# Linyou/Ced-NeRF

Measured on NVIDIA B200. Metric: train_step_rays_per_s, higher is better.
Workload: dtype f16 (MLP, tables) / f32 (marching, compositing, grads)

## Files before the change

cednerf_b200/_lib.py:

```python
from __future__ import annotations

import ctypes
import os
from typing import Optional

import torch

_HERE = os.path.dirname(os.path.abspath(__file__))
LIB_PATH = os.environ.get("CEDNERF_B200_LIB") or os.path.join(_HERE, "libcednerf_b200.so")

MAX_LEVELS = 32
MLP_MAX_LAYERS = 5


class GridLevels(ctypes.Structure):
    _fields_ = [("n_levels", ctypes.c_int), ("scale", ctypes.c_float * MAX_LEVELS),
                ("res", ctypes.c_uint32 * MAX_LEVELS), ("size", ctypes.c_uint32 * MAX_LEVELS),
                ("offset", ctypes.c_uint32 * MAX_LEVELS), ("hashed", ctypes.c_uint32 * MAX_LEVELS)]


class MlpDesc(ctypes.Structure):
    _fields_ = [("n_layers", ctypes.c_int), ("dim_in", ctypes.c_int * MLP_MAX_LAYERS),
                ("dim_out", ctypes.c_int * MLP_MAX_LAYERS), ("param_off", ctypes.c_int * MLP_MAX_LAYERS),
                ("image_off", ctypes.c_int * MLP_MAX_LAYERS), ("image_bytes", ctypes.c_int)]
# ... 39 lines not shown
class DpSmall(ctypes.Structure):
    _fields_ = [("world", ctypes.c_int), ("n_tensors", ctypes.c_int), ("grad", ctypes.c_void_p * DP_MAX_RANKS),
                ("p", ctypes.c_void_p * 8), ("m", ctypes.c_void_p * 8), ("v", ctypes.c_void_p * 8),
                ("off", ctypes.c_int64 * 8), ("n", ctypes.c_int64 * 8), ("lr", ctypes.c_float * 8),
                ("weight_decay", ctypes.c_float * 8), ("grad_div", ctypes.c_float), ("chunk_begin", ctypes.c_int64 * 9)]


class RenderRound(ctypes.Structure):
    _P, _I, _L, _F = ctypes.c_void_p, ctypes.c_int, ctypes.c_int64, ctypes.c_float
    _fields_ = [("rays_o", _P), ("rays_d", _P), ("n_rays", _L), ("occ_bits", _P), ("aabbs", _P), ("n_levels", _I),
                ("resolution", _I), ("near_term", _P), ("far_const", _F), ("step_size", _F), ("cone_angle", _F),
                ("early_stop_eps", _F), ("t_sorted", _P), ("t_indices", _P), ("hits", _P), ("state", _P), ("total", _P),
                ("n_samples", _P), ("run_t", _P), ("run_n", _P), ("n_runs", _P), ("occ_coarse", _P), ("capacity", _L),
                ("offsets", _P), ("totals", _P), ("scan_workspace", _P), ("t_starts", _P), ("t_ends", _P),
                ("ray_indices", _P), ("overflow", _P), ("timestamps", _P), ("image_deform", _P), ("image_density", _P),
                ("image_colour", _P), ("table_f16", _P), ("desc", ctypes.POINTER(FieldDesc)), ("sigma", _P), ("rgbs", _P),
                ("colors", _P), ("opacity", _P), ("depth", _P), ("alive_flags", _P), ("positions", _P),
                ("position_totals", _P), ("run_cap", _I), ("k_hint", _I), ("max_samples", _I), ("min_samples", _I)]


_SIGNATURES = {
    "cednerf_ray_aabb_intersect": "pplpifffpppp",
    "cednerf_sort_boundaries": "pplippp",
    "cednerf_occ_pack_bits": "plpp",
    "cednerf_occ_threshold_pack": "plpppp",
    "cednerf_occ_mark_invisible": "pipiipiiiifpp",
    "cednerf_march": "ipplppiippffffippppppppppppppppppppppippp",
    "cednerf_occ_coarsen": "piipp",
    "cednerf_ray_coherence_keys": "plpp",
    "cednerf_ray_coherence_order": "plppp",
    "cednerf_march_fill_runs": "lppppiffppppp",
    "cednerf_exclusive_scan": "plppppp",
    "cednerf_exclusive_scan_capped": "pllpppp",
    "cednerf_march_fill_runs_capped": "lpppppiffppppp",
    "cednerf_compact_samples_capped": "pppppllpppp",
    "cednerf_hashgrid_fwd": "pilpGpip",
    "cednerf_hashgrid_bwd": "pilpGpiippp",
    "cednerf_hashgrid_bwd_table_lm": "pilGppp",
    "cednerf_hashgrid4d_fwd": "pilpGpiip",
    "cednerf_hashgrid4d_bwd": "pilGpiipip",
    "cednerf_cast_f32_to_f16": "pplp",
    "cednerf_frequency_fwd": "pilipiifp",
    "cednerf_frequency_bwd": "pilipiipp",
    "cednerf_sh2_fwd": "plpip",
    "cednerf_time_embed": "pplpp",
    "cednerf_mlp_pack_weights": "pMpp",
    "cednerf_mlp_fwd": "ppMlppp",
    "cednerf_mlp_bwd": "ppppMlpippp",
    "cednerf_field_fwd": "ppppppppilppppFpppp",
    "cednerf_occ_update_level": "plpppiffpppFpppp",
    "cednerf_field_train_fwd": "ppppppilpppppFppppppppp",
    "cednerf_field_train_bwd": "ppppppilpppppFpppppppppppppippp",
    "cednerf_sample_order": "ppppplpffffffppp",
    "cednerf_ray_offsets": "pllpp",
    "cednerf_composite_fwd": "pppppppillpppppppifp",
    "cednerf_composite_bwd": "pppppppillppppppppppfp",
    "cednerf_visibility_mask": "ppppllffppp",
    "cednerf_compact_samples": "pppppllpppp",
    "cednerf_accumulate_fwd": "ppipllpip",
    "cednerf_accumulate_bwd": "ppiplppppp",
    "cednerf_render_round_begin": "pliippp",
    "cednerf_march_round": "ipplppiipfffppppppppppppppipp",
    "cednerf_march_fill_runs_round": "lpppppiffppppppp",
    "cednerf_render_round_composite": "pppppppplifppppp",
    "cednerf_render_round_compact":"ppplppliippp",
    "cednerf_render_round": "Rlppp",
    "cednerf_generate_rays": "ppppiffffiilpppp",
    "cednerf_distortion_fwd": "pppplpppp",
    "cednerf_distortion_bwd": "pppplpppp",
    "cednerf_importance_keys": "ppplpp",
    "cednerf_topk_select": "pllpppp",
    "cednerf_importance_batch": "pliiippiffffipppppppp",
    "cednerf_nonfinite_check": "App",
    "cednerf_training_loss_fwd": "ppplppplpiffpppp",
    "cednerf_training_loss_bwd": "pppplpppliffpppppp",
    "cednerf_adam_step": "Apippfffip",
    "cednerf_peer_alloc": "lp",
    "cednerf_peer_free": "p",
    "cednerf_ipc_export": "pp",
    "cednerf_ipc_open": "pp",
    "cednerf_ipc_close": "p",
    "cednerf_dp_barrier": "Puip",
    "cednerf_dp_found_inf": "Pppp",
    "cednerf_dp_adam": "Dpppfffip",
    "cednerf_dp_adam_small": "Spppfffip",
}
_CT = {"p": ctypes.c_void_p, "i": ctypes.c_int, "l": ctypes.c_int64, "f": ctypes.c_float,
       "G": ctypes.POINTER(GridLevels), "M": ctypes.POINTER(MlpDesc), "F": ctypes.POINTER(FieldDesc),
       "A": ctypes.POINTER(AdamTensors), "P": ctypes.POINTER(DpPeers), "D": ctypes.POINTER(DpAdam), "S": ctypes.POINTER(DpSmall),
       "u": ctypes.c_uint32, "R": ctypes.POINTER(RenderRound)}

_lib = None


def load() -> ctypes.CDLL:
    global _lib
    if _lib is not None:
        return _lib
    if not os.path.exists(LIB_PATH):
        raise ImportError(
            f"{LIB_PATH} is missing: build it with `make -C cednerf_b200/csrc` (or `python -c 'import "
            "__graft_entry__ as g; g.build()'`).  cednerf_b200 has no CPU / PyTorch fallback.")
    lib = ctypes.CDLL(LIB_PATH)
    lib.cednerf_last_error.restype = ctypes.c_char_p
    lib.cednerf_scan_workspace_bytes.restype = ctypes.c_int64
    lib.cednerf_launch_count.restype = ctypes.c_int64
# ... 78 lines not shown
```

cednerf_b200/csrc/field_train.cu:

```cuda
#include <stdlib.h>

#include "field_common.cuh"

namespace {

struct SavedLayout {
  int64_t h1, o1, in2, h2, o2, h3, h4, o4, xn, total, tiles;
};

__host__ __device__ inline SavedLayout saved_layout(const CednerfFieldDesc& d, int64_t n) {
  SavedLayout s;
  int64_t off = 0;
  const int64_t tiles = (n + MLP_TILE - 1) / MLP_TILE;
  s.tiles = tiles;
  s.h1 = off, off += (int64_t)(d.f1.n_layers - 1) * tiles * MLP_TILE_BYTES;
  s.o1 = off, off += n * 32;
  s.in2 = off, off += n * d.f2.dim_in[0] * 2;
  s.h2 = off, off += (int64_t)(d.f2.n_layers - 1) * tiles * MLP_TILE_BYTES;
  s.o2 = off, off += n * 32;
  s.h3 = off, off += (int64_t)(d.f3.n_layers - 1) * tiles * MLP_TILE_BYTES;
  s.h4 = off, off += d.f4.n_layers > 0 ? (int64_t)(d.f4.n_layers - 1) * tiles * MLP_TILE_BYTES : 0;
  s.o4 = off, off += d.f4.n_layers > 0 ? n * 64 : 0;
  s.xn = off, off += (n * 12 + 15) / 16 * 16;
  s.total = off;
  return s;
}

struct BwdWorkLayout {
  int64_t d_o2, d_in2, d_in4, g_xn, dy_lm, total;
};

__host__ __device__ inline BwdWorkLayout bwd_layout(const CednerfFieldDesc& d, int64_t n) {
  BwdWorkLayout w;
  int64_t off = 0;
  w.d_o2 = off, off += n * 32;
  w.d_in2 = off, off += n * d.f2.dim_in[0] * 2;
  w.d_in4 = off, off += n * 64;
  w.g_xn = off, off += (n * 12 + 15) / 16 * 16;
  w.dy_lm = off, off += (int64_t)d.levels.n_levels * n * 4;
  w.total = off;
  return w;
}

struct TrainArgs {
  const int64_t* ridx;
  const float* t0;
  const float* t1;
  const float* rays_o;
  const float* rays_d;
  const float* t;
  int t_stride;
  int64_t n;
  const int64_t* n_dev;
  const uint8_t* img[4];
  const __half* table;
  float* sigma;
  float* rgb;
  float* latent;
  uint8_t* selector;
  float* move;
  uint8_t* saved;
  const float* d_sigma;
  const float* d_rgb;
  const float* d_latent;
  uint8_t* work;
  float* d_params[4];
  uint32_t tmem_cols;
  int flush_tiles;
  const int32_t* order;
  CednerfFieldDesc d;
};

__device__ __forceinline__ int64_t ext_index(const TrainArgs& a, int64_t s) { return a.order ? (int64_t)a.order[s] : s; }

__device__ __forceinline__ int64_t live_count(const TrainArgs& a) {
  if (!a.n_dev) return a.n;
  const int64_t v = *a.n_dev;
  return v < a.n ? v : a.n;
}

__device__ __forceinline__ float huber(float x) {
  const float ax = fabsf(x);
  return ax < 1.f ? 0.5f * x * x : ax - 0.5f;
}

__device__ __forceinline__ void load_off(const TrainArgs& a, const SavedLayout& sl, int64_t s, float* off6) {
  const uint4 w = *reinterpret_cast<const uint4*>(a.saved + sl.o1 + s * 32);
  const uint32_t ww[4] = {w.x, w.y, w.z, w.w};
#pragma unroll
// ... 27 lines not shown
__global__ void __launch_bounds__(TRAIN_FWD_GROUPS * 128, 1) field_train_fwd_kernel(TrainArgs a) {
  extern __shared__ __align__(1024) uint8_t smem_raw[];
  uint8_t* smem = reinterpret_cast<uint8_t*>((reinterpret_cast<uintptr_t>(smem_raw) + 1023) & ~(uintptr_t)1023);
  const CednerfFieldDesc& d = a.d;
  const bool has4 = d.f4.n_layers > 0;
  const int n_groups = blockDim.x / MLP_TILE;
  const int tid = threadIdx.x, warp = tid >> 5, group = tid / MLP_TILE, gtid = tid % MLP_TILE;
  uint8_t* w1 = smem;
  uint8_t* w2 = w1 + d.f1.image_bytes;
  uint8_t* w3 = w2 + d.f2.image_bytes;
  uint8_t* w4 = w3 + d.f3.image_bytes;
  uint8_t* abuf = reinterpret_cast<uint8_t*>(
                      (reinterpret_cast<uintptr_t>(w4 + (has4 ? d.f4.image_bytes : 0)) + 1023) & ~(uintptr_t)1023) +
                  (size_t)group * MLP_TILE_BYTES;
  __shared__ uint64_t bars[8];
  __shared__ uint32_t tmem_base_s;
  uint64_t* bar = &bars[group];
  {
    const uint8_t* src[4] = {a.img[0], a.img[1], a.img[2], a.img[3]};
    uint8_t* dst[4] = {w1, w2, w3, w4};
    const int bytes[4] = {d.f1.image_bytes, d.f2.image_bytes, d.f3.image_bytes, has4 ? d.f4.image_bytes : 0};
    for (int k = 0; k < 4; ++k)
      for (int q = tid; q < bytes[k] / 16; q += blockDim.x)
        reinterpret_cast<uint4*>(dst[k])[q] = __ldg(reinterpret_cast<const uint4*>(src[k]) + q);
  }
  const uint32_t tmem_cols = n_groups <= 1 ? 64 : (n_groups == 2 ? 128 : (n_groups <= 4 ? 256 : 512));
  if (warp == 0) tmem_alloc(&tmem_base_s, tmem_cols);
  if (gtid == 0) mbar_init(bar, 1);
  if (tid == 0) fence_barrier_init();
  fence_proxy_async();
  tc_fence_before();
  __syncthreads();
  tc_fence_after();
  const uint32_t tmem_base = tmem_base_s + 64u * (uint32_t)group;
  const uint32_t tmem_warp = tmem_base + ((uint32_t)((warp & 3) * 32) << 16);
  uint32_t phase = 0;
  const int64_t n = a.n, nl = live_count(a);
  const int64_t n_tiles = (nl + MLP_TILE - 1) / MLP_TILE;
  const int L = d.levels.n_levels;
  const uint32_t one2 = 0x3C003C00u;
  const SavedLayout sl = saved_layout(d, n);
  const int k2 = d.f2.dim_in[0];

  for (int64_t tile = blockIdx.x + (int64_t)gridDim.x * group; tile < n_tiles; tile += (int64_t)gridDim.x * n_groups) {
    const int64_t s = tile * MLP_TILE + gtid;
    const bool ok = s < nl;
    const int rows_valid = (int)((nl - tile * MLP_TILE) < MLP_TILE ? (nl - tile * MLP_TILE) : MLP_TILE);
    float x[3] = {0.f, 0.f, 0.f}, tv = 0.f;
    int64_t ray = 0;
#ifdef FIELD_PHASE_CLOCKS
    long long phase_t = clock64();
    if (gtid == 0) atomicAdd(&g_train_phase_clocks[11], 1ull);
#endif
    const int64_t e = ok ? ext_index(a, s) : 0;
    if (ok) packed_sample(a.ridx, a.t0, a.t1, a.rays_o, a.rays_d, a.t, a.t_stride, e, x, tv, ray);
    frequency_row<true>(abuf, gtid, x[0], x[1], x[2], tv);
    fence_proxy_async();
    tc_fence_before();
    group_sync(group);
    TPHASE_MARK(0);
    run_chain(d.f1, w1, abuf, tmem_base, tmem_warp, bar, phase, gtid, group, a.saved + sl.h1,
              sl.tiles, tile * MLP_TILE, rows_valid);
    TPHASE_MARK(1);
    float xn[3], mv[3], mvnorm;
    bool selector;
    {
      uint32_t r[16];
      tmem_ld16(tmem_warp, r);
      tmem_ld_wait();
      uint32_t p[8];
#pragma unroll
      for (int j = 0; j < 8; ++j) p[j] = pack_h2(__uint_as_float(r[2 * j]), __uint_as_float(r[2 * j + 1]));
      if (ok) {
        uint4* dst = reinterpret_cast<uint4*>(a.saved + sl.o1 + s * 32);
        dst[0] = make_uint4(p[0], p[1], p[2], p[3]);
        dst[1] = make_uint4(p[4], p[5], p[6], p[7]);
      }
      float off6[6];
#pragma unroll
      for (int k = 0; k < 6; ++k) off6[k] = rnd16(r[k]);
      apply_move(d, x, off6, mv, xn, selector);
      mvnorm = sqrtf(mv[0] * mv[0] + mv[1] * mv[1] + mv[2] * mv[2]);
    }
    if (ok) {
      float* xs = reinterpret_cast<float*>(a.saved + sl.xn) + 3 * s;
      xs[0] = xn[0], xs[1] = xn[1], xs[2] = xn[2];
      a.move[3 * e] = mv[0], a.move[3 * e + 1] = mv[1], a.move[3 * e + 2] = mv[2];
      a.selector[e] = (uint8_t)selector;
    }
    TPHASE_MARK(2);
    float temb[9];
    {
      auto put_word = [&](int w, uint32_t v) {
        *reinterpret_cast<uint32_t*>(abuf + swz(gtid, w >> 2) + ((w & 3) << 2)) = v;
      };
      if ((L % TRAIN_FWD_LG) == 0 && (L & 3) == 0) {
#pragma unroll 1
        for (int l0 = 0; l0 < L; l0 += TRAIN_FWD_LG) {
          uint32_t fw[TRAIN_FWD_LG];
          hash_levels<TRAIN_FWD_LG>(xn, a.table, d.levels, 0, fw, l0);
          if constexpr (TRAIN_FWD_LG >= 4) {
#pragma unroll
            for (int q = 0; q < TRAIN_FWD_LG / 4; ++q)
              *reinterpret_cast<uint4*>(abuf + swz(gtid, (l0 >> 2) + q)) = make_uint4(fw[4 * q], fw[4 * q + 1], fw[4 * q + 2], fw[4 * q + 3]);
          } else {
            *reinterpret_cast<uint2*>(abuf + swz(gtid, l0 >> 2) + ((l0 & 2) << 2)) = make_uint2(fw[0], fw[1]);
          }
        }
// ... 117 lines not shown
__device__ __forceinline__ void predictor_dout(const TrainArgs& a, const SavedLayout& sl, int64_t s, int cb, uint32_t* dw) {
  const int k2 = a.d.f2.dim_in[0];
  const uint4* ps = reinterpret_cast<const uint4*>(a.saved + sl.o4 + s * 64) + 2 * cb;
  const uint4* fs = reinterpret_cast<const uint4*>(a.saved + sl.in2 + s * k2 * 2) + 2 * cb;
  const int64_t e = ext_index(a, s);
  const bool sel = a.selector[e] != 0;
#pragma unroll
  for (int c = 0; c < 2; ++c) {
    const uint4 p = ps[c], f = fs[c];
    const uint32_t pw[4] = {p.x, p.y, p.z, p.w}, fw[4] = {f.x, f.y, f.z, f.w};
    const float4 l0 = *reinterpret_cast<const float4*>(a.d_latent + e * 32 + (2 * cb + c) * 8);
    const float4 l1 = *reinterpret_cast<const float4*>(a.d_latent + e * 32 + (2 * cb + c) * 8 + 4);
    const float lg[8] = {l0.x, l0.y, l0.z, l0.w, l1.x, l1.y, l1.z, l1.w};
#pragma unroll
    for (int j = 0; j < 4; ++j) {
      const float2 pv = __half22float2(*reinterpret_cast<const __half2*>(&pw[j]));
      const float2 fv = __half22float2(*reinterpret_cast<const __half2*>(&fw[j]));
      const float d0 = sel ? lg[2 * j] * fminf(fmaxf(pv.x - fv.x, -1.f), 1.f) : 0.f;
      const float d1 = sel ? lg[2 * j + 1] * fminf(fmaxf(pv.y - fv.y, -1.f), 1.f) : 0.f;
      dw[4 * c + j] = pack_h2(d0, d1);
    }
  }
}

template <int NET>
__device__ __forceinline__ void make_dout(const TrainArgs& a, const SavedLayout& sl, const BwdWorkLayout& wl, uint8_t* tile,
                                          int row, int64_t s, bool ok) {
  const CednerfFieldDesc& d = a.d;
  uint32_t w[16];
#pragma unroll
  for (int j = 0; j < 16; ++j) w[j] = 0u;
  const int n_chunks = NET == 4 ? 4 : 2;
  if (ok) {
    if constexpr (NET == 3) {
      float g[3];
#pragma unroll
      for (int k = 0; k < 3; ++k) {
        const int64_t e = ext_index(a, s);
        const float c = a.rgb[3 * e + k];
        g[k] = a.d_rgb[3 * e + k] * c * (1.f - c);
      }
      w[0] = pack_h2(g[0], g[1]);
      w[1] = pack_h2(g[2], 0.f);
    } else if constexpr (NET == 2) {
      const uint4* src = reinterpret_cast<const uint4*>(a.work + wl.d_o2 + s * 32);
      const uint4 g0 = src[0], g1 = src[1];
      w[0] = g0.x, w[1] = g0.y, w[2] = g0.z, w[3] = g0.w, w[4] = g1.x, w[5] = g1.y, w[6] = g1.z, w[7] = g1.w;
      const __half raw = *reinterpret_cast<const __half*>(a.saved + sl.o2 + s * 32);
      const int64_t e = ext_index(a, s);
      const float gs = a.selector[e] ? a.d_sigma[e] * expf(fminf(__half2float(raw) - 1.f, 15.f)) : 0.f;
      const float hi = __half2float(__ushort_as_half((unsigned short)(w[0] >> 16)));
      w[0] = pack_h2(gs, hi);
    } else if constexpr (NET == 4) {
      predictor_dout(a, sl, s, 0, w);
      predictor_dout(a, sl, s, 1, w + 8);
    } else {
      const float* gx = reinterpret_cast<const float*>(a.work + wl.g_xn) + 3 * s;
      float g[3] = {gx[0], gx[1], gx[2]};
      if (d.f4.n_layers > 0 && a.d_latent) {
        const float* xs = reinterpret_cast<const float*>(a.saved + sl.xn) + 3 * s;
        const uint4* src = reinterpret_cast<const uint4*>(a.work + wl.d_in4 + s * 64);
#pragma unroll
        for (int dim = 0; dim < 3; ++dim) {
          const uint4 q = src[dim];
          const uint32_t qw[4] = {q.x, q.y, q.z, q.w};
          float acc = 0.f;
#pragma unroll
          for (int k = 0; k < 4; ++k) {
            const float2 gv = __half22float2(*reinterpret_cast<const __half2*>(&qw[k]));
            const float sc = (float)(1 << k);
            float sn, cs;
            sincospi_fast(xs[dim] * sc, sn, cs);
            acc += (gv.x * cs - gv.y * sn) * sc * 3.14159265358979323846f;
          }
          g[dim] += acc;
        }
      }
      float off6[6];
      load_off(a, sl, s, off6);
      float o[6] = {0.f, 0.f, 0.f, 0.f, 0.f, 0.f};
#pragma unroll
      for (int k = 0; k < 3; ++k) {
        const float gm = g[k] / (d.aabb[3 + k] - d.aabb[k]);
        o[k] = gm * d.moving_step;
        if (d.use_div_offsets) {
          const float th = tanhf(off6[3 + k]);
          o[3 + k] = gm * d.moving_step * (1.f - th * th);
        }
      }
      w[0] = pack_h2(o[0], o[1]);
      w[1] = pack_h2(o[2], o[3]);
      w[2] = pack_h2(o[4], o[5]);
    }
  }
#pragma unroll
  for (int c = 0; c < 4; ++c)
    if (c < n_chunks) *reinterpret_cast<uint4*>(tile + swz(row, c)) = make_uint4(w[4 * c], w[4 * c + 1], w[4 * c + 2], w[4 * c + 3]);
}

template <int NET>
__device__ __forceinline__ void make_input(const TrainArgs& a, const SavedLayout& sl, uint8_t* tile, int row, int64_t s,
                                           bool ok) {
  const CednerfFieldDesc& d = a.d;
  if (!ok) {
    const int chunks = net_desc<NET>(d).dim_in[0] / 8;
    for (int c = 0; c < chunks; ++c) *reinterpret_cast<uint4*>(tile + swz(row, c)) = make_uint4(0u, 0u, 0u, 0u);
    return;
  }
  if constexpr (NET == 2) {
    const int k2 = d.f2.dim_in[0];
    const uint4* src = reinterpret_cast<const uint4*>(a.saved + sl.in2 + s * k2 * 2);
    for (int c = 0; c < k2 / 8; ++c) *reinterpret_cast<uint4*>(tile + swz(row, c)) = src[c];
    return;
  }
  float x[3], tv;
  int64_t ray;
  packed_sample(a.ridx, a.t0, a.t1, a.rays_o, a.rays_d, a.t, a.t_stride, ext_index(a, s), x, tv, ray);
  if constexpr (NET == 1) {
    frequency_row<true>(tile, row, x[0], x[1], x[2], tv);
  } else if constexpr (NET == 4) {
    const float* xs = reinterpret_cast<const float*>(a.saved + sl.xn) + 3 * s;
    frequency_row<true>(tile, row, xs[0], xs[1], xs[2], tv);
  } else {
    float temb[9];
    if (d.time_mode && !d.time_before_sigma) {
      float off6[6], mv[3], xn[3];
      bool sel;
      load_off(a, sl, s, off6);
      apply_move(d, x, off6, mv, xn, sel);
      time_embedding<true>(tv, sqrtf(mv[0] * mv[0] + mv[1] * mv[1] + mv[2] * mv[2]), d.time_mode, temb);
    }
    const uint4* src = reinterpret_cast<const uint4*>(a.saved + sl.o2 + s * 32);
    const uint4 q0 = src[0], q1 = src[1];
    const uint32_t qw[8] = {q0.x, q0.y, q0.z, q0.w, q1.x, q1.y, q1.z, q1.w};
    float o2[16];
#pragma unroll
    for (int j = 0; j < 8; ++j) {
      const float2 f = __half22float2(*reinterpret_cast<const __half2*>(&qw[j]));
      o2[2 * j] = f.x, o2[2 * j + 1] = f.y;
    }
    const float dir[3] = {a.rays_d[3 * ray], a.rays_d[3 * ray + 1], a.rays_d[3 * ray + 2]};
    colour_input_row(d, tile, row, dir, o2 + 1, temb);
  }
}

#define BWD_GROUPS 4
#define BWD_GROUP_SMEM (3 * MLP_TILE_BYTES)

template <int NET>
__global__ void __launch_bounds__(BWD_GROUPS * MLP_TILE, 1) field_bwd_kernel(TrainArgs a) {
  extern __shared__ __align__(1024) uint8_t smem_raw[];
  uint8_t* smem = reinterpret_cast<uint8_t*>((reinterpret_cast<uintptr_t>(smem_raw) + 1023) & ~(uintptr_t)1023);
  const CednerfMlpDesc& d = net_desc<NET>(a.d);
  const int n_groups = blockDim.x / MLP_TILE;
  const int tid = threadIdx.x, warp = tid >> 5, lane = tid & 31, group = tid / MLP_TILE, gtid = tid % MLP_TILE;
  uint8_t* wsm = smem;
  uint8_t* gsm = smem + ((d.image_bytes + 1023) & ~1023) + (size_t)group * BWD_GROUP_SMEM;
  uint8_t* gbuf = gsm;
  uint8_t* ibuf[2] = {gsm + MLP_TILE_BYTES, gsm + 2 * MLP_TILE_BYTES};
  __shared__ uint64_t bars[BWD_GROUPS];
  __shared__ uint32_t tmem_base_s;
  uint64_t* bar = &bars[group];
  const int64_t n = a.n, nl = live_count(a);
  const SavedLayout sl = saved_layout(a.d, n);
  const BwdWorkLayout wl = bwd_layout(a.d, n);
  const uint8_t* image = a.img[NET - 1];
  const uint8_t* hidden = a.saved + (NET == 1 ? sl.h1 : (NET == 2 ? sl.h2 : (NET == 3 ? sl.h3 : sl.h4)));
  __shared__ uint64_t lbars[BWD_GROUPS];
  uint64_t* lbar = &lbars[group];
  uint32_t lphase = 0;
// ... 111 lines not shown
          for (int k = 0; k < N_out / 16; ++k) umma(tmem_grp, ad + 2 * k, bd + 128 * k, id, k > 0);
        }
        umma_commit(bar);
      }
      if (l > 0) {
        if (l > 1) fetch_tile(ibuf[cur ^ 1], l - 2, tile);
        else make_input<NET>(a, sl, ibuf[cur ^ 1], gtid, s, ok);
      }
      if ((gtid >> 5) == 0) {
        mbar_wait(bar, phase);
        tc_fence_after();
        tc_fence_before();
      }
      group_sync(group);
      phase ^= 1;
      tc_fence_after();
      if (l > 0) {
        const uint8_t* act = ibuf[cur];
#pragma unroll
        for (int cb = 0; cb < 4; ++cb) {
          uint32_t r[16];
          tmem_ld16(tmem_warp + cb * 16, r);
          tmem_ld_wait();
          const uint4 m0 = *reinterpret_cast<const uint4*>(act + swz(gtid, 2 * cb));
          const uint4 m1 = *reinterpret_cast<const uint4*>(act + swz(gtid, 2 * cb + 1));
          const uint32_t mw[8] = {m0.x, m0.y, m0.z, m0.w, m1.x, m1.y, m1.z, m1.w};
          uint32_t p[8];
#pragma unroll
          for (int j = 0; j < 8; ++j) {
            const unsigned keep = __hgt2_mask(*reinterpret_cast<const __half2*>(&mw[j]), __float2half2_rn(0.f));
            p[j] = pack_h2(__uint_as_float(r[2 * j]), __uint_as_float(r[2 * j + 1])) & keep;
          }
          *reinterpret_cast<uint4*>(gbuf + swz(gtid, 2 * cb)) = make_uint4(p[0], p[1], p[2], p[3]);
          *reinterpret_cast<uint4*>(gbuf + swz(gtid, 2 * cb + 1)) = make_uint4(p[4], p[5], p[6], p[7]);
        }
      } else if (want_dx) {
        if constexpr (NET == 3) {
          uint32_t r0[16], r1[16];
          tmem_ld16(tmem_warp, r0);
          tmem_ld16(tmem_warp + 16, r1);
          tmem_ld_wait();
          if (ok) {
            float v[16];
            v[0] = 0.f;
#pragma unroll
            for (int j = 1; j <= 12; ++j) v[j] = __uint_as_float(r0[3 + j]);
#pragma unroll
            for (int j = 13; j <= 15; ++j) v[j] = __uint_as_float(r1[j - 13]);
            uint4* dst = reinterpret_cast<uint4*>(a.work + wl.d_o2 + s * 32);
            dst[0] = make_uint4(pack_h2(v[0], v[1]), pack_h2(v[2], v[3]), pack_h2(v[4], v[5]), pack_h2(v[6], v[7]));
            dst[1] = make_uint4(pack_h2(v[8], v[9]), pack_h2(v[10], v[11]), pack_h2(v[12], v[13]), pack_h2(v[14], v[15]));
          }
        } else {
          uint8_t* out = a.work + (NET == 2 ? wl.d_in2 + s * K_in * 2 : wl.d_in4 + s * 64);
          for (int cb = 0; cb < K_in / 16; ++cb) {
            uint32_t r[16];
            tmem_ld16(tmem_warp + cb * 16, r);
            tmem_ld_wait();
            if (ok) {
              uint32_t p[8];
#pragma unroll
              for (int j = 0; j < 8; ++j) p[j] = pack_h2(__uint_as_float(r[2 * j]), __uint_as_float(r[2 * j + 1]));
              if constexpr (NET == 2) {
                if (a.d.f4.n_layers > 0 && a.d_latent && cb < 2) {
                  uint32_t dw[8];
                  predictor_dout(a, sl, s, cb, dw);
#pragma unroll
                  for (int j = 0; j < 8; ++j) {
                    const __half2 q = __hsub2(*reinterpret_cast<const __half2*>(&p[j]), *reinterpret_cast<const __half2*>(&dw[j]));
                    p[j] = *reinterpret_cast<const uint32_t*>(&q);
                  }
                }
                uint32_t* lm = reinterpret_cast<uint32_t*>(a.work + wl.dy_lm);
#pragma unroll
                for (int j = 0; j < 8; ++j)
                  if (8 * cb + j < a.d.levels.n_levels) lm[(int64_t)(8 * cb + j) * n + s] = p[j];
              } else {
                reinterpret_cast<uint4*>(out)[2 * cb] = make_uint4(p[0], p[1], p[2], p[3]);
                reinterpret_cast<uint4*>(out)[2 * cb + 1] = make_uint4(p[4], p[5], p[6], p[7]);
              }
            }
          }
        }
      }
      if (l > 1) await_tile();
      fence_proxy_async();
      tc_fence_before();
      group_sync(group);
      cur ^= 1;
    }
  }
  tc_fence_before();
  __syncthreads();
  tc_fence_after();
  flush_wgrad(false);
  __syncthreads();
  if (warp == 0) tmem_dealloc(tmem_base, a.tmem_cols);
}

__global__ void __launch_bounds__(256) hashgrid_bwd_input_lm_kernel(const float* __restrict__ xn, int64_t n,
                                                                    const __half* __restrict__ table, CednerfGridLevels lv,
                                                                    const __half2* __restrict__ dy_lm, float* __restrict__ g_x,
                                                                    const int64_t* __restrict__ n_dev) {
  const int64_t s = (int64_t)blockIdx.x * blockDim.x + threadIdx.x;
  if (s >= n || (n_dev && s >= *n_dev)) return;
  const float x[3] = {xn[3 * s], xn[3 * s + 1], xn[3 * s + 2]};
  float gx[3] = {0.f, 0.f, 0.f};
  const int L = lv.n_levels;
  auto level_terms = [&](const float* f, const __half2* v, int l) {
    const float2 d = __half22float2(dy_lm[(int64_t)l * n + s]);
    float dot[8];
#pragma unroll
    for (int k = 0; k < 8; ++k) {
      const float2 t = __half22float2(v[k]);
      dot[k] = t.x * d.x + t.y * d.y;
    }
    const float wx[2] = {1.f - f[0], f[0]}, wy[2] = {1.f - f[1], f[1]}, wz[2] = {1.f - f[2], f[2]};
    float a[3] = {0.f, 0.f, 0.f};
#pragma unroll
// ... 187 lines not shown
```

cednerf_b200/csrc/sample_order.cu:

```cuda
#include "common.cuh"

#define SO_BITS 7
#define SO_BINS (1 << (3 * SO_BITS))
#define SO_BLOCK 1024
#define SO_BLOCKS (SO_BINS / SO_BLOCK)
#define SO_RANK_MAX 512u

namespace {

__device__ __forceinline__ uint32_t spread3(uint32_t v) {
  v = (v | (v << 16)) & 0x030000FFu;
  v = (v | (v << 8)) & 0x0300F00Fu;
  v = (v | (v << 4)) & 0x030C30C3u;
  v = (v | (v << 2)) & 0x09249249u;
  return v;
}

__device__ __forceinline__ int64_t live_of(int64_t n, const int64_t* n_dev) {
  if (!n_dev) return n;
  const int64_t v = *n_dev;
  return v < n ? v : n;
}

__global__ void so_keys_kernel(const int64_t* __restrict__ ridx, const float* __restrict__ t0, const float* __restrict__ t1,
// ... 33 lines not shown
#pragma unroll
    for (int o = 1; o < 32; o <<= 1) {
      const uint32_t u = __shfl_up_sync(0xffffffffu, t, o);
      if (lane >= o) t += u;
    }
    ws[lane] = t;
  }
  __syncthreads();
  hist[blockIdx.x * SO_BLOCK + threadIdx.x] = (warp ? ws[warp - 1] : 0u) + incl - v;
  if (threadIdx.x == SO_BLOCK - 1) totals[blockIdx.x] = ws[31];
}

__global__ void __launch_bounds__(1024) so_totals_scan_kernel(uint32_t* __restrict__ totals) {
  __shared__ uint32_t ws[32];
  const int lane = threadIdx.x & 31, warp = threadIdx.x >> 5;
  const uint32_t a = totals[2 * threadIdx.x], b = totals[2 * threadIdx.x + 1];
  uint32_t incl = a + b;
#pragma unroll
  for (int o = 1; o < 32; o <<= 1) {
    const uint32_t u = __shfl_up_sync(0xffffffffu, incl, o);
    if (lane >= o) incl += u;
  }
  if (lane == 31) ws[warp] = incl;
  __syncthreads();
  if (warp == 0) {
    uint32_t t = ws[lane];
#pragma unroll
    for (int o = 1; o < 32; o <<= 1) {
      const uint32_t u = __shfl_up_sync(0xffffffffu, t, o);
      if (lane >= o) t += u;
    }
    ws[lane] = t;
  }
  __syncthreads();
  const uint32_t excl = (warp ? ws[warp - 1] : 0u) + incl - (a + b);
  totals[2 * threadIdx.x] = excl;
  totals[2 * threadIdx.x + 1] = excl + a;
}

__global__ void so_scatter_kernel(const uint32_t* __restrict__ keys, int64_t n, const int64_t* __restrict__ n_dev,
                                  uint32_t* __restrict__ cursor, const uint32_t* __restrict__ totals,
                                  int32_t* __restrict__ unordered, uint32_t* __restrict__ slot_of) {
  const int64_t s = (int64_t)blockIdx.x * blockDim.x + threadIdx.x;
  if (s >= live_of(n, n_dev)) return;
  const uint32_t key = keys[s];
  const uint32_t p = atomicAdd(&cursor[key], 1u) + totals[key / SO_BLOCK];
  unordered[p] = (int32_t)s;
  slot_of[s] = p;
}

__global__ void so_rank_kernel(const uint32_t* __restrict__ keys, int64_t n, const int64_t* __restrict__ n_dev,
                               const uint32_t* __restrict__ cursor, const uint32_t* __restrict__ totals,
                               const int32_t* __restrict__ unordered, const uint32_t* __restrict__ slot_of,
                               int32_t* __restrict__ order) {
  const int64_t s = (int64_t)blockIdx.x * blockDim.x + threadIdx.x;
  if (s >= n) return;
  if (s >= live_of(n, n_dev)) {
    order[s] = (int32_t)s;
    return;
  }
  const uint32_t key = keys[s], base = totals[key / SO_BLOCK];
  const uint32_t lo = base + ((key % SO_BLOCK) ? cursor[key - 1] : 0u), hi = base + cursor[key];
  if (hi - lo > SO_RANK_MAX) {
    order[slot_of[s]] = (int32_t)s;
    return;
  }
  uint32_t rank = 0;
  for (uint32_t p = lo; p < hi; ++p) rank += unordered[p] < (int32_t)s;
  order[lo + rank] = (int32_t)s;
}

}

CEDNERF_EXPORT int64_t cednerf_sample_order_workspace_bytes(int64_t n) {
  return (int64_t)SO_BINS * 4 + SO_BLOCKS * 4 + 3 * ((n + 3) / 4 * 16);
}

CEDNERF_EXPORT int cednerf_sample_order(const int64_t* ray_indices, const float* t_starts, const float* t_ends,
                                        const float* rays_o, const float* rays_d, int64_t n, const int64_t* n_device,
                                        float lo0, float lo1, float lo2, float hi0, float hi1, float hi2, void* workspace,
                                        int32_t* order, void* stream) {
  CEDNERF_REQUIRE(n >= 0 && n < (1ll << 31) && ray_indices && t_starts && t_ends && rays_o && rays_d && workspace && order,
                  "bad arguments");
  CEDNERF_REQUIRE(hi0 > lo0 && hi1 > lo1 && hi2 > lo2, "empty box");
  if (n == 0) return 0;
  cudaStream_t st = (cudaStream_t)stream;
  uint32_t* hist = (uint32_t*)workspace;
  uint32_t* totals = hist + SO_BINS;
  uint32_t* keys = totals + SO_BLOCKS;
  cudaMemsetAsync(hist, 0, (size_t)SO_BINS * 4, st);
  const float cells = (float)(1 << SO_BITS);
  so_keys_kernel<<<cednerf_blocks(n, 256), 256, 0, st>>>(ray_indices, t_starts, t_ends, rays_o, rays_d, n, n_device, lo0, lo1,
                                                         lo2, cells / (hi0 - lo0), cells / (hi1 - lo1), cells / (hi2 - lo2),
                                                         keys, hist);
  so_block_scan_kernel<<<SO_BLOCKS, SO_BLOCK, 0, st>>>(hist, totals);
  so_totals_scan_kernel<<<1, 1024, 0, st>>>(totals);
  int32_t* unordered = (int32_t*)(keys + (n + 3) / 4 * 4);
  uint32_t* slot_of = (uint32_t*)(unordered + (n + 3) / 4 * 4);
  so_scatter_kernel<<<cednerf_blocks(n, 256), 256, 0, st>>>(keys, n, n_device, hist, totals, unordered, slot_of);
  so_rank_kernel<<<cednerf_blocks(n, 256), 256, 0, st>>>(keys, n, n_device, hist, totals, unordered, slot_of, order);
  return cednerf_check_launch("cednerf_sample_order", 5);
}
```

cednerf_b200/ops.py:

```python
from __future__ import annotations

import ctypes
import math
from typing import List, Optional, Sequence, Tuple

import torch

from . import _lib
from ._lib import FieldDesc, GridLevels, MlpDesc, call, ptr, stream

F32, F16, I64, I32, U8 = torch.float32, torch.float16, torch.int64, torch.int32, torch.uint8


def _f32c(t: torch.Tensor) -> torch.Tensor:
    _lib.check_device()
    if not t.is_cuda:
        raise RuntimeError("cednerf_b200 ops need CUDA tensors (no CPU fallback)")
    return t.detach().to(F32).contiguous()


def ray_aabb_intersect(rays_o, rays_d, aabbs, near_plane=-math.inf, far_plane=math.inf, miss_value=math.inf):
    o, d, bx = _f32c(rays_o), _f32c(rays_d), _f32c(aabbs)
    n, nl = o.shape[0], bx.shape[0]
    t_mins = torch.empty(n, nl, device=o.device)
# ... 583 lines not shown
    if packed is not None:
        ridx, t0, t1, o, d = packed
        ridx_c, t0_c, t1_c, o_c, d_c = ridx.detach().to(I64).contiguous(), _f32c(t0), _f32c(t1), _f32c(o), _f32c(d)
        args = (ptr(ridx_c), ptr(t0_c), ptr(t1_c), ptr(o_c), ptr(d_c), None, None)
    else:
        x, dirs = points
        xs = _f32c(x)
        ds = None if dirs is None else _f32c(dirs)
        args = (None, None, None, None, None, ptr(xs), ptr(ds))
    call("cednerf_field_fwd", *args, ptr(ts), int(t_stride), n, ptr(images[0]), ptr(images[1]), ptr(images[2]),
         ptr(table_f16), ctypes.byref(desc), ptr(sigma), ptr(rgb), ptr(n_dev), stream())
    del args
    return sigma, rgb


_table_grad_hook = None

SAMPLE_ORDER_MIN = None


def set_table_grad_hook(fn):
    global _table_grad_hook
    _table_grad_hook = fn


_table_grad_alloc = None


def set_table_grad_alloc(fn):
    global _table_grad_alloc
    _table_grad_alloc = fn


class FieldTrainFunction(torch.autograd.Function):

    @staticmethod
    def forward(ctx, p1, p2, p3, p4, table, desc, images, table_f16, ridx, t0, t1, rays_o, rays_d, ts, t_stride,
                want_latent, n_dev=None, order_box=None):
        _lib.check_device()
        lib = _lib.load()
        n, dev = t0.numel(), t0.device
        ridx = ridx.detach().to(I64).contiguous()
        t0, t1, rays_o, rays_d = _f32c(t0), _f32c(t1), _f32c(rays_o), _f32c(rays_d)
        ts = _f32c(ts).view(-1)
        sigma = _sempty(n, device=dev)
        rgb = _sempty(n, 3, device=dev)
        latent = _sempty(n, 32, device=dev) if want_latent else None
        selector = _sempty(n, dtype=torch.bool, device=dev)
        move = _sempty(n, 3, device=dev)
        saved = torch.empty(max(int(lib.cednerf_field_saved_bytes(ctypes.byref(desc), _sticky_capacity(n))), 16), dtype=U8, device=dev)
        order = None
        if SAMPLE_ORDER_MIN is not None and n >= SAMPLE_ORDER_MIN:
            order = _sempty(n, dtype=torch.int32, device=dev)
            ws = torch.empty(int(lib.cednerf_sample_order_workspace_bytes(_sticky_capacity(n))), dtype=U8, device=dev)
            bx = [float(v) for v in (order_box if order_box is not None else desc.aabb)]
            call("cednerf_sample_order", ptr(ridx), ptr(t0), ptr(t1), ptr(rays_o), ptr(rays_d), n, ptr(n_dev), *bx,
                 ptr(ws), ptr(order), stream())
        call("cednerf_field_train_fwd", ptr(ridx), ptr(t0), ptr(t1), ptr(rays_o), ptr(rays_d), ptr(ts), int(t_stride), n,
             ptr(images[0]), ptr(images[1]), ptr(images[2]), ptr(images[3]), ptr(table_f16), ctypes.byref(desc),
             ptr(sigma), ptr(rgb), ptr(latent), ptr(selector), ptr(move), ptr(saved), ptr(order), ptr(n_dev), stream())
        ctx.order = order
        ctx.save_for_backward(ridx, t0, t1, rays_o, rays_d, ts, sigma, rgb, selector, saved, table_f16, images[0],
                              images[1], images[2], images[3] if images[3] is not None else images[0])
        ctx.desc, ctx.t_stride, ctx.has4 = desc, int(t_stride), images[3] is not None and want_latent
        ctx.n_dev = n_dev
        ctx.shapes = (p1.shape, p2.shape, p3.shape, None if p4 is None else p4.shape, table.shape)
        ctx.mark_non_differentiable(selector, move)
        ctx.set_materialize_grads(False)
        if latent is None:
            latent = torch.zeros(0, device=dev)
        return sigma, rgb, latent, selector, move

    @staticmethod
    def backward(ctx, d_sigma, d_rgb, d_latent, _sel, _mv):
        note_parameter_gradient()
        ridx, t0, t1, rays_o, rays_d, ts, sigma, rgb, selector, saved, table_f16, i1, i2, i3, i4 = ctx.saved_tensors
        lib = _lib.load()
        n, dev = t0.numel(), t0.device
        s1, s2, s3, s4, st = ctx.shapes
        want4 = ctx.has4 and s4 is not None
        sizes = [math.prod(s) for s in (s1, s2, s3)] + ([math.prod(s4)] if want4 else [])
        padded = [(k + 3) // 4 * 4 for k in sizes]
        pool = torch.zeros(sum(padded), dtype=F32, device=dev)
        views, o = [], 0
        for k, kp, shp in zip(sizes, padded, (s1, s2, s3) + ((s4,) if want4 else ())):
            views.append(pool[o:o + k].view(shp))
            o += kp
        g1, g2, g3 = views[:3]
        g4 = views[3] if want4 else None
        gt = _table_grad_alloc(st, dev) if _table_grad_alloc is not None else None
        if gt is None:
            gt = torch.zeros(st, dtype=F32, device=dev)
        d_sigma = torch.zeros(n, device=dev) if d_sigma is None else _f32c(d_sigma)
        d_rgb = torch.zeros(n, 3, device=dev) if d_rgb is None else _f32c(d_rgb)
        dl = None
        if ctx.has4 and d_latent is not None and d_latent.numel():
            dl = _f32c(d_latent)
        work = torch.empty(max(int(lib.cednerf_field_bwd_workspace_bytes(ctypes.byref(ctx.desc), _sticky_capacity(n))), 16), dtype=U8,
                           device=dev)
        hook = _table_grad_hook
        for phase in ((1, 2) if hook is not None else (0,)):
            if n:
                call("cednerf_field_train_bwd", ptr(ridx), ptr(t0), ptr(t1), ptr(rays_o), ptr(rays_d), ptr(ts),
                     ctx.t_stride, n, ptr(i1), ptr(i2), ptr(i3), ptr(i4) if ctx.has4 else None, ptr(table_f16),
                     ctypes.byref(ctx.desc), ptr(sigma), ptr(rgb), ptr(selector), ptr(saved), ptr(d_sigma), ptr(d_rgb),
                     ptr(dl), ptr(work), ptr(g1), ptr(g2), ptr(g3), ptr(g4) if dl is not None else None, ptr(gt), phase,
                     ptr(ctx.order), ptr(ctx.n_dev), stream())
            if phase == 1:
                hook(gt)
        return (g1, g2, g3, g4 if dl is not None else None, gt) + (None,) * 13
# ... 1 lines not shown
```

include/cednerf_b200.h:

```cpp
#ifndef CEDNERF_B200_H
#define CEDNERF_B200_H

#include <stdint.h>

#ifdef __cplusplus
extern "C" {
#endif

#define CEDNERF_ERR_BAD_ARG (-1)
#define CEDNERF_ERR_UNSUPPORTED (-2)

#define CEDNERF_MAX_LEVELS 32
#define CEDNERF_MLP_MAX_LAYERS 5

const char* cednerf_last_error(void);
int cednerf_abi_version(void);
int cednerf_check_device(void);
int64_t cednerf_launch_count(void);

int cednerf_ray_aabb_intersect(const float* rays_o, const float* rays_d, int64_t n_rays, const float* aabbs,
                               int n_levels, float near_plane, float far_plane, float miss_value, float* t_mins,
                               float* t_maxs, uint8_t* hits, void* stream);
int cednerf_sort_boundaries(const float* t_mins, const float* t_maxs, int64_t n_rays, int n_levels, float* t_sorted,
                            int64_t* t_indices, void* stream);
// ... 74 lines not shown
int cednerf_mlp_bwd(const void* x_f16, const void* hidden_f16, const void* d_out_f16, const void* weight_image,
                    const CednerfMlpDesc* desc, int64_t n, void* d_x , int dx_is_f32,
                    float* d_params ,
                    void* d_hidden_f16 ,
                    void* stream);

typedef struct CednerfFieldDesc {
  float aabb[6];
  float moving_step;
  int use_div_offsets;
  int time_mode;
  int time_before_sigma;
  CednerfMlpDesc f1, f2, f3;
  CednerfMlpDesc f4;
  CednerfGridLevels levels;
} CednerfFieldDesc;
int cednerf_field_fwd(const int64_t* ray_indices, const float* t_starts, const float* t_ends, const float* rays_o,
                      const float* rays_d, const float* x, const float* dirs, const float* timestamps, int t_stride,
                      int64_t n, const void* image_deform, const void* image_density, const void* image_colour,
                      const void* table_f16, const CednerfFieldDesc* desc, float* sigma, float* rgb,
                      const int64_t* n_device , void* stream);

int cednerf_occ_update_level(const int64_t* cells , int64_t n, const float* jitter ,
                             const float* timestamps , const float* level_aabb , int resolution,
                             float step_scale, float ema_decay, const void* image_deform, const void* image_density,
                             const void* table_f16, const CednerfFieldDesc* desc, float* occs_level,
                             float* cand , uint8_t* touched , void* stream);

int64_t cednerf_field_saved_bytes(const CednerfFieldDesc* desc, int64_t n);
int64_t cednerf_field_bwd_workspace_bytes(const CednerfFieldDesc* desc, int64_t n);
int cednerf_field_train_fwd(const int64_t* ray_indices, const float* t_starts, const float* t_ends, const float* rays_o,
                            const float* rays_d, const float* timestamps, int t_stride, int64_t n,
                            const void* image_deform, const void* image_density, const void* image_colour,
                            const void* image_predict, const void* table_f16, const CednerfFieldDesc* desc, float* sigma,
                            float* rgb, float* latent, uint8_t* selector, float* move, void* saved,
                            const int32_t* sample_order ,
                            const int64_t* n_device ,
                            void* stream);
int cednerf_field_train_bwd(const int64_t* ray_indices, const float* t_starts, const float* t_ends, const float* rays_o,
                            const float* rays_d, const float* timestamps, int t_stride, int64_t n,
                            const void* image_deform, const void* image_density, const void* image_colour,
                            const void* image_predict, const void* table_f16, const CednerfFieldDesc* desc,
                            const float* sigma, const float* rgb, const uint8_t* selector, const void* saved,
                            const float* d_sigma, const float* d_rgb, const float* d_latent, void* work,
                            float* d_params_deform, float* d_params_density, float* d_params_colour,
                            float* d_params_predict, float* g_table, int phase,
                            const int32_t* sample_order ,
                            const int64_t* n_device , void* stream);

int64_t cednerf_sample_order_workspace_bytes(int64_t n);
int cednerf_sample_order(const int64_t* ray_indices, const float* t_starts, const float* t_ends, const float* rays_o,
                         const float* rays_d, int64_t n, const int64_t* n_device, float lo0, float lo1, float lo2,
                         float hi0, float hi1, float hi2, void* workspace, int32_t* order, void* stream);

int cednerf_ray_offsets(const int64_t* ray_indices, int64_t n_samples, int64_t n_rays, int64_t* offsets, void* stream);
int cednerf_composite_fwd(const float* t_starts, const float* t_ends, const float* sigmas, const float* rgbs,
                          const float* prefix_trans, const int64_t* offsets, const float* bkgd, int bkgd_stride,
                          int64_t n_samples, int64_t n_rays, float* weights, float* trans, float* alphas,
                          float* colors, float* opacity, float* depth, float* depth_raw, int accumulate_inplace,
                          float depth_eps, void* stream);
int cednerf_composite_bwd(const float* t_starts, const float* t_ends, const float* rgbs, const float* trans,
                          const float* alphas, const int64_t* offsets, const float* bkgd, int bkgd_stride,
                          int64_t n_samples, int64_t n_rays, const float* opacity, const float* depth_raw,
                          const float* g_colors, const float* g_opacity, const float* g_depth, const float* g_weights,
                          const float* g_trans, const float* g_alphas, float* g_sigmas, float* g_rgbs, float depth_eps,
                          void* stream);
int cednerf_visibility_mask(const float* t_starts, const float* t_ends, const float* sigmas, const int64_t* offsets,
                            int64_t n_samples, int64_t n_rays, float early_stop_eps, float alpha_thre, uint8_t* keep,
                            int32_t* kept_counts , void* stream);
int cednerf_compact_samples(const uint8_t* keep, const int64_t* offsets, const int64_t* out_starts, const float* t_starts,
                            const float* t_ends, int64_t n_samples, int64_t n_rays, int64_t* ray_indices_out,
                            float* t_starts_out, float* t_ends_out, void* stream);
int cednerf_compact_samples_capped(const uint8_t* keep, const int64_t* offsets, const int64_t* out_offsets,
                                   const float* t_starts, const float* t_ends, int64_t n_samples, int64_t n_rays,
                                   int64_t* ray_indices_out, float* t_starts_out, float* t_ends_out, void* stream);
int cednerf_render_round_begin(int32_t* state, int64_t n_rays, int max_samples, int min_samples,
                               const int64_t* prev_totals , int64_t* total ,
                               void* stream);
int cednerf_march_round(int fill, const float* rays_o, const float* rays_d, int64_t n_bound, const uint32_t* occ_bits,
                        const float* aabbs, int n_levels, int resolution, float* near_term , float far_const, float step_size, float cone_angle,
                        const float* t_sorted, const int64_t* t_indices, const uint8_t* hits, const int32_t* alive,
                        const int32_t* state, const uint8_t* slot_mask , const int64_t* offsets ,
                        float* t_starts, float* t_ends, int64_t* ray_indices, int32_t* n_samples ,
                        float* run_t, int32_t* run_n, int32_t* n_runs, int run_cap,
                        const uint32_t* occ_coarse , void* stream);
int cednerf_march_fill_runs_round(int64_t n_bound, const int64_t* offsets, const int32_t* n_samples, const float* run_t,
                                  const int32_t* run_n, const int32_t* n_runs, int run_cap, float step_size,
                                  float cone_angle, const int32_t* alive, const int32_t* state, float* t_starts,
                                  float* t_ends, int64_t* ray_indices, uint8_t* overflow, void* stream);
int cednerf_render_round_composite(const float* t_starts, const float* t_ends, const float* sigmas, const float* rgbs,
                                   const int64_t* offsets, const int32_t* alive, int32_t* round_state,
                                   const int32_t* slot_counts, int64_t n_bound, int k_hint, float early_stop_eps,
                                   float* colors, float* opacity, float* depth, int32_t* alive_flags ,
                                   void* stream);
int cednerf_render_round_compact(const int32_t* alive_flags, const int64_t* positions, const int32_t* alive,
                                 int64_t n_bound, int32_t* round_state, int32_t* next_alive, int64_t n_rays,
                                 int max_samples ,
                                 int min_samples, const int64_t* round_totals, int64_t* total, void* stream);
typedef struct CednerfRenderRound {
  const float* rays_o;
  const float* rays_d;
  int64_t n_rays;
  const uint32_t* occ_bits;
  const float* aabbs;
  int n_levels, resolution;
  float* near_term;
// ... 150 lines not shown
```

Before: 54.26 million.

## Gather sample ray/t arrays into walk order and cache predictor output grads

The sample-order rank kernel now also writes ray indices and t_start/t_end permuted into the spatial walk order, so the field train kernels read them contiguously by position instead of through the order indirection. The backward colour pass stores the predictor output gradients into a new work buffer slot (replacing the unused d_in2 slot), and the NET==4 backward reads them back rather than recomputing predictor_dout. This removes scattered gathers and some recomputation, at the cost of extra permuted arrays and more workspace memory. It depends on NET==2 backward running before NET==4 so the buffer is filled, and on the ordered path being enabled when n reaches SAMPLE_ORDER_MIN.

```diff
diff --git a/cednerf_b200/_lib.py b/cednerf_b200/_lib.py
--- a/cednerf_b200/_lib.py
+++ b/cednerf_b200/_lib.py
@@ -115,6 +115,7 @@
     "cednerf_field_train_fwd": "ppppppilpppppFppppppppp",
     "cednerf_field_train_bwd": "ppppppilpppppFpppppppppppppippp",
     "cednerf_sample_order": "ppppplpffffffppp",
+    "cednerf_sample_walk": "ppppplpffffffpppppp",
     "cednerf_ray_offsets": "pllpp",
     "cednerf_composite_fwd": "pppppppillpppppppifp",
     "cednerf_composite_bwd": "pppppppillppppppppppfp",
diff --git a/cednerf_b200/csrc/field_train.cu b/cednerf_b200/csrc/field_train.cu
--- a/cednerf_b200/csrc/field_train.cu
+++ b/cednerf_b200/csrc/field_train.cu
@@ -27,14 +27,14 @@
 }
 
 struct BwdWorkLayout {
-  int64_t d_o2, d_in2, d_in4, g_xn, dy_lm, total;
+  int64_t d_o2, d_o4, d_in4, g_xn, dy_lm, total;
 };
 
 __host__ __device__ inline BwdWorkLayout bwd_layout(const CednerfFieldDesc& d, int64_t n) {
   BwdWorkLayout w;
   int64_t off = 0;
   w.d_o2 = off, off += n * 32;
-  w.d_in2 = off, off += n * d.f2.dim_in[0] * 2;
+  w.d_o4 = off, off += d.f4.n_layers > 0 ? n * 64 : 0;
   w.d_in4 = off, off += n * 64;
   w.g_xn = off, off += (n * 12 + 15) / 16 * 16;
   w.dy_lm = off, off += (int64_t)d.levels.n_levels * n * 4;
@@ -168,8 +168,8 @@
     long long phase_t = clock64();
     if (gtid == 0) atomicAdd(&g_train_phase_clocks[11], 1ull);
 #endif
+    if (ok) packed_sample(a.ridx, a.t0, a.t1, a.rays_o, a.rays_d, a.t, a.t_stride, s, x, tv, ray);
     const int64_t e = ok ? ext_index(a, s) : 0;
-    if (ok) packed_sample(a.ridx, a.t0, a.t1, a.rays_o, a.rays_d, a.t, a.t_stride, e, x, tv, ray);
     frequency_row<true>(abuf, gtid, x[0], x[1], x[2], tv);
     fence_proxy_async();
     tc_fence_before();
@@ -393,8 +393,12 @@
       const float hi = __half2float(__ushort_as_half((unsigned short)(w[0] >> 16)));
       w[0] = pack_h2(gs, hi);
     } else if constexpr (NET == 4) {
-      predictor_dout(a, sl, s, 0, w);
-      predictor_dout(a, sl, s, 1, w + 8);
+      const uint4* src = reinterpret_cast<const uint4*>(a.work + wl.d_o4 + s * 64);
+#pragma unroll
+      for (int c = 0; c < 4; ++c) {
+        const uint4 q = src[c];
+        w[4 * c] = q.x, w[4 * c + 1] = q.y, w[4 * c + 2] = q.z, w[4 * c + 3] = q.w;
+      }
     } else {
       const float* gx = reinterpret_cast<const float*>(a.work + wl.g_xn) + 3 * s;
       float g[3] = {gx[0], gx[1], gx[2]};
@@ -456,7 +460,7 @@
   }
   float x[3], tv;
   int64_t ray;
-  packed_sample(a.ridx, a.t0, a.t1, a.rays_o, a.rays_d, a.t, a.t_stride, ext_index(a, s), x, tv, ray);
+  packed_sample(a.ridx, a.t0, a.t1, a.rays_o, a.rays_d, a.t, a.t_stride, s, x, tv, ray);
   if constexpr (NET == 1) {
     frequency_row<true>(tile, row, x[0], x[1], x[2], tv);
   } else if constexpr (NET == 4) {
@@ -674,7 +678,7 @@
             dst[1] = make_uint4(pack_h2(v[8], v[9]), pack_h2(v[10], v[11]), pack_h2(v[12], v[13]), pack_h2(v[14], v[15]));
           }
         } else {
-          uint8_t* out = a.work + (NET == 2 ? wl.d_in2 + s * K_in * 2 : wl.d_in4 + s * 64);
+          uint8_t* out = a.work + (NET == 2 ? wl.d_o4 : wl.d_in4) + s * 64;
           for (int cb = 0; cb < K_in / 16; ++cb) {
             uint32_t r[16];
             tmem_ld16(tmem_warp + cb * 16, r);
@@ -687,6 +691,8 @@
                 if (a.d.f4.n_layers > 0 && a.d_latent && cb < 2) {
                   uint32_t dw[8];
                   predictor_dout(a, sl, s, cb, dw);
+                  reinterpret_cast<uint4*>(out)[2 * cb] = make_uint4(dw[0], dw[1], dw[2], dw[3]);
+                  reinterpret_cast<uint4*>(out)[2 * cb + 1] = make_uint4(dw[4], dw[5], dw[6], dw[7]);
 #pragma unroll
                   for (int j = 0; j < 8; ++j) {
                     const __half2 q = __hsub2(*reinterpret_cast<const __half2*>(&p[j]), *reinterpret_cast<const __half2*>(&dw[j]));
diff --git a/cednerf_b200/csrc/sample_order.cu b/cednerf_b200/csrc/sample_order.cu
--- a/cednerf_b200/csrc/sample_order.cu
+++ b/cednerf_b200/csrc/sample_order.cu
@@ -109,7 +109,9 @@
 __global__ void so_rank_kernel(const uint32_t* __restrict__ keys, int64_t n, const int64_t* __restrict__ n_dev,
                                const uint32_t* __restrict__ cursor, const uint32_t* __restrict__ totals,
                                const int32_t* __restrict__ unordered, const uint32_t* __restrict__ slot_of,
-                               int32_t* __restrict__ order) {
+                               int32_t* __restrict__ order, const int64_t* __restrict__ ridx, const float* __restrict__ t0,
+                               const float* __restrict__ t1, int64_t* __restrict__ w_ridx, float* __restrict__ w_t0,
+                               float* __restrict__ w_t1) {
   const int64_t s = (int64_t)blockIdx.x * blockDim.x + threadIdx.x;
   if (s >= n) return;
   if (s >= live_of(n, n_dev)) {
@@ -118,13 +120,16 @@
   }
   const uint32_t key = keys[s], base = totals[key / SO_BLOCK];
   const uint32_t lo = base + ((key % SO_BLOCK) ? cursor[key - 1] : 0u), hi = base + cursor[key];
+  uint32_t p;
   if (hi - lo > SO_RANK_MAX) {
-    order[slot_of[s]] = (int32_t)s;
-    return;
+    p = slot_of[s];
+  } else {
+    uint32_t rank = 0;
+    for (uint32_t q = lo; q < hi; ++q) rank += unordered[q] < (int32_t)s;
+    p = lo + rank;
   }
-  uint32_t rank = 0;
-  for (uint32_t p = lo; p < hi; ++p) rank += unordered[p] < (int32_t)s;
-  order[lo + rank] = (int32_t)s;
+  order[p] = (int32_t)s;
+  if (w_ridx) w_ridx[p] = ridx[s], w_t0[p] = t0[s], w_t1[p] = t1[s];
 }
 
 }
@@ -133,15 +138,16 @@
   return (int64_t)SO_BINS * 4 + SO_BLOCKS * 4 + 3 * ((n + 3) / 4 * 16);
 }
 
-CEDNERF_EXPORT int cednerf_sample_order(const int64_t* ray_indices, const float* t_starts, const float* t_ends,
-                                        const float* rays_o, const float* rays_d, int64_t n, const int64_t* n_device,
-                                        float lo0, float lo1, float lo2, float hi0, float hi1, float hi2, void* workspace,
-                                        int32_t* order, void* stream) {
+namespace {
+
+int sample_order(const int64_t* ray_indices, const float* t_starts, const float* t_ends, const float* rays_o,
+                 const float* rays_d, int64_t n, const int64_t* n_device, float lo0, float lo1, float lo2, float hi0,
+                 float hi1, float hi2, void* workspace, int32_t* order, int64_t* w_ridx, float* w_t0, float* w_t1,
+                 cudaStream_t st, const char* name) {
   CEDNERF_REQUIRE(n >= 0 && n < (1ll << 31) && ray_indices && t_starts && t_ends && rays_o && rays_d && workspace && order,
                   "bad arguments");
   CEDNERF_REQUIRE(hi0 > lo0 && hi1 > lo1 && hi2 > lo2, "empty box");
   if (n == 0) return 0;
-  cudaStream_t st = (cudaStream_t)stream;
   uint32_t* hist = (uint32_t*)workspace;
   uint32_t* totals = hist + SO_BINS;
   uint32_t* keys = totals + SO_BLOCKS;
@@ -155,6 +161,27 @@
   int32_t* unordered = (int32_t*)(keys + (n + 3) / 4 * 4);
   uint32_t* slot_of = (uint32_t*)(unordered + (n + 3) / 4 * 4);
   so_scatter_kernel<<<cednerf_blocks(n, 256), 256, 0, st>>>(keys, n, n_device, hist, totals, unordered, slot_of);
-  so_rank_kernel<<<cednerf_blocks(n, 256), 256, 0, st>>>(keys, n, n_device, hist, totals, unordered, slot_of, order);
-  return cednerf_check_launch("cednerf_sample_order", 5);
+  so_rank_kernel<<<cednerf_blocks(n, 256), 256, 0, st>>>(keys, n, n_device, hist, totals, unordered, slot_of, order,
+                                                         ray_indices, t_starts, t_ends, w_ridx, w_t0, w_t1);
+  return cednerf_check_launch(name, 5);
 }
+
+}
+
+CEDNERF_EXPORT int cednerf_sample_order(const int64_t* ray_indices, const float* t_starts, const float* t_ends,
+                                        const float* rays_o, const float* rays_d, int64_t n, const int64_t* n_device,
+                                        float lo0, float lo1, float lo2, float hi0, float hi1, float hi2, void* workspace,
+                                        int32_t* order, void* stream) {
+  return sample_order(ray_indices, t_starts, t_ends, rays_o, rays_d, n, n_device, lo0, lo1, lo2, hi0, hi1, hi2, workspace,
+                      order, nullptr, nullptr, nullptr, (cudaStream_t)stream, "cednerf_sample_order");
+}
+
+CEDNERF_EXPORT int cednerf_sample_walk(const int64_t* ray_indices, const float* t_starts, const float* t_ends,
+                                       const float* rays_o, const float* rays_d, int64_t n, const int64_t* n_device,
+                                       float lo0, float lo1, float lo2, float hi0, float hi1, float hi2, void* workspace,
+                                       int32_t* order, int64_t* walk_ray_indices, float* walk_t_starts,
+                                       float* walk_t_ends, void* stream) {
+  CEDNERF_REQUIRE(walk_ray_indices && walk_t_starts && walk_t_ends, "bad arguments");
+  return sample_order(ray_indices, t_starts, t_ends, rays_o, rays_d, n, n_device, lo0, lo1, lo2, hi0, hi1, hi2, workspace,
+                      order, walk_ray_indices, walk_t_starts, walk_t_ends, (cudaStream_t)stream, "cednerf_sample_walk");
+}
diff --git a/cednerf_b200/ops.py b/cednerf_b200/ops.py
--- a/cednerf_b200/ops.py
+++ b/cednerf_b200/ops.py
@@ -659,10 +659,12 @@
         order = None
         if SAMPLE_ORDER_MIN is not None and n >= SAMPLE_ORDER_MIN:
             order = _sempty(n, dtype=torch.int32, device=dev)
+            w_ridx, w_t0, w_t1 = _sempty(n, dtype=I64, device=dev), _sempty(n, device=dev), _sempty(n, device=dev)
             ws = torch.empty(int(lib.cednerf_sample_order_workspace_bytes(_sticky_capacity(n))), dtype=U8, device=dev)
             bx = [float(v) for v in (order_box if order_box is not None else desc.aabb)]
-            call("cednerf_sample_order", ptr(ridx), ptr(t0), ptr(t1), ptr(rays_o), ptr(rays_d), n, ptr(n_dev), *bx,
-                 ptr(ws), ptr(order), stream())
+            call("cednerf_sample_walk", ptr(ridx), ptr(t0), ptr(t1), ptr(rays_o), ptr(rays_d), n, ptr(n_dev), *bx,
+                 ptr(ws), ptr(order), ptr(w_ridx), ptr(w_t0), ptr(w_t1), stream())
+            ridx, t0, t1 = w_ridx, w_t0, w_t1
         call("cednerf_field_train_fwd", ptr(ridx), ptr(t0), ptr(t1), ptr(rays_o), ptr(rays_d), ptr(ts), int(t_stride), n,
              ptr(images[0]), ptr(images[1]), ptr(images[2]), ptr(images[3]), ptr(table_f16), ctypes.byref(desc),
              ptr(sigma), ptr(rgb), ptr(latent), ptr(selector), ptr(move), ptr(saved), ptr(order), ptr(n_dev), stream())
diff --git a/include/cednerf_b200.h b/include/cednerf_b200.h
--- a/include/cednerf_b200.h
+++ b/include/cednerf_b200.h
@@ -150,6 +150,10 @@
 int cednerf_sample_order(const int64_t* ray_indices, const float* t_starts, const float* t_ends, const float* rays_o,
                          const float* rays_d, int64_t n, const int64_t* n_device, float lo0, float lo1, float lo2,
                          float hi0, float hi1, float hi2, void* workspace, int32_t* order, void* stream);
+int cednerf_sample_walk(const int64_t* ray_indices, const float* t_starts, const float* t_ends, const float* rays_o,
+                        const float* rays_d, int64_t n, const int64_t* n_device, float lo0, float lo1, float lo2,
+                        float hi0, float hi1, float hi2, void* workspace, int32_t* order, int64_t* walk_ray_indices,
+                        float* walk_t_starts, float* walk_t_ends, void* stream);
 
 int cednerf_ray_offsets(const int64_t* ray_indices, int64_t n_samples, int64_t n_rays, int64_t* offsets, void* stream);
 int cednerf_composite_fwd(const float* t_starts, const float* t_ends, const float* sigmas, const float* rgbs,
```

Result: faster. 54.86 million, median of 6 (+1.1%).
